# pierrepaleo/sift_pyocl

Measured on AMD Instinct MI355X. Metric: SiftPlan.keypoints throughput, 4096x4096 fp32 (Mpix/s; keypoints/s in keypoints_per_s), higher is better.
Workload: dtype f32

## Files before the change

sift_pyocl_amd/csrc/k_keypoint.hpp:

```cpp
#pragma once
#include <hip/hip_runtime.h>
#include <stdint.h>
#include "k_extrema.hpp"
#include "siftmath.hpp"

namespace siftk {

struct KpRecord { float x, y, scale, angle; uint8_t desc[128]; };
static_assert(sizeof(KpRecord) == 144, "record layout");

struct GradTaps { float xa, xb, ya, yb; bool bx, by; };

__device__ __forceinline__ GradTaps gradient_fetch(const float *__restrict__ I, int x, int y, int W, int H) {
    const size_t pos = (size_t)y * W + x;
    GradTaps t;
    t.bx = (x == 0) || (x == W - 1);
    t.by = (y == 0) || (y == H - 1);
    t.xa = I[x == W - 1 ? pos : pos + 1];
    t.xb = I[x == 0 ? pos : pos - 1];
    t.ya = I[y == 0 ? pos : pos - W];
    t.yb = I[y == H - 1 ? pos : pos + W];
    return t;
}

__device__ __forceinline__ void gradient_eval(const GradTaps &t, float &mag, float &ori) {
    float gx = t.xa - t.xb, gy = t.ya - t.yb;
    if (t.bx) gx = 2.0f * gx;
    if (t.by) gy = 2.0f * gy;
    mag = sqrtf(gx * gx + gy * gy);
    ori = siftmath::atan2f_(-gy, gx);
}

__device__ __forceinline__ void gradient_at(const float *__restrict__ I, int x, int y, int W, int H,
                                            float &mag, float &ori) {
    gradient_eval(gradient_fetch(I, x, y, W, H), mag, ori);
}

__device__ __forceinline__ int div_exact(int idx, int d, float inv, int &rem) {
    int q = (int)((float)idx * inv);
    rem = idx - q * d;
    if (rem < 0) { q--; rem += d; }
    else if (rem >= d) { q++; rem -= d; }
    return q;
}

#define SIFT_MAX_OCTAVES 24
#define SIFT_GROUPS 3
struct Counters {
    int n_rec;
    int tail_timeout;
    unsigned rec_word[SIFT_GROUPS];
    int g_kp[SIFT_GROUPS];
    int g_out[SIFT_GROUPS];
    int desc_next[SIFT_GROUPS];
    int n_cand[SIFT_MAX_OCTAVES + 1];
    int c_scale[SIFT_MAX_OCTAVES][3];
    int o_scale[SIFT_MAX_OCTAVES][3];
    uint32_t mm[2];
    int tail_ready[8];
};

struct OctaveTable {
    const float *base;
    long long off[SIFT_MAX_OCTAVES];
    int W[SIFT_MAX_OCTAVES], H[SIFT_MAX_OCTAVES];
    const float *gmap, *omap;
};
__device__ __forceinline__ size_t map_offset(const OctaveTable &tab, int oct, int scale) {
    return (size_t)(tab.off[oct] / 2) + (size_t)(scale - 1) * tab.W[oct] * tab.H[oct];
}

struct alignas(16) RecordSink {
    KpRecord *dev, *host;
    int dev_limit, host_limit;
};

__device__ __forceinline__ void descriptor_open(Counters *cnt, int group, int n, KpRecord *records, int rec_capacity, KpRecord *host_records,
                                                int host_capacity, RecordSink *S) {
    if (threadIdx.x == 0) {
        int base = 0;
        if (cnt) {
            if (blockIdx.x == 0) {
                base = atomicAdd(&cnt->n_rec, n);
                __hip_atomic_store(&cnt->rec_word[group], 0x80000000u | (unsigned)base, __ATOMIC_RELAXED, __HIP_MEMORY_SCOPE_AGENT);
            } else {
                unsigned w;
                while (!((w = __hip_atomic_load(&cnt->rec_word[group], __ATOMIC_RELAXED, __HIP_MEMORY_SCOPE_AGENT)) & 0x80000000u)) __builtin_amdgcn_s_sleep(16);
                base = (int)(w & 0x7fffffffu);
            }
        }
        S->dev = records + base; S->dev_limit = rec_capacity - base;
        S->host = host_records ? host_records + base : nullptr; S->host_limit = host_records ? host_capacity - base : 0;
    }
    __syncthreads();
}

__device__ __forceinline__ void store_record(const RecordSink *S, int i, const float4 kq, int b0, int b1, int lane, unsigned char *bytes) {
    bytes[lane] = (unsigned char)b0; bytes[lane + 64] = (unsigned char)b1;
    __builtin_amdgcn_wave_barrier();
    unsigned w = 0u;
    if (lane < 4) w = __float_as_uint(lane == 0 ? kq.x : (lane == 1 ? kq.y : (lane == 2 ? kq.z : kq.w)));
    else if (lane < 36) w = reinterpret_cast<const unsigned *>(bytes)[lane - 4];
    if (lane < 36) {
        const volatile RecordSink *v = S;
        if (i < v->dev_limit) reinterpret_cast<unsigned *>(v->dev + i)[lane] = w;
        if (i < v->host_limit) reinterpret_cast<unsigned *>(v->host + i)[lane] = w;
    }
    __builtin_amdgcn_wave_barrier();
}

__global__ void gather_records_kernel(const KpRecord *__restrict__ records, const int *__restrict__ idx, KpRecord *__restrict__ out, int n) {
    const long long total = (long long)n * 36;
    for (long long t = (long long)blockIdx.x * blockDim.x + threadIdx.x; t < total; t += (long long)gridDim.x * blockDim.x) {
        const int j = (int)(t / 36), w = (int)(t - (long long)j * 36);
        reinterpret_cast<unsigned *>(out + j)[w] = reinterpret_cast<const unsigned *>(records + idx[j])[w];
    }
}

#ifdef SIFT_PHASE_CLOCK
__device__ unsigned long long g_phase[32];
struct PhaseClock {
    unsigned long long t, t0;
    unsigned long long *acc;
    __device__ __forceinline__ void start(unsigned long long *lds16, int lane) {
        acc = lds16;
        if (lane < 16) lds16[lane] = 0ull;
        __builtin_amdgcn_wave_barrier();
        t0 = t = __builtin_amdgcn_s_memtime();
    }
    __device__ __forceinline__ void mark(int k, int lane) {
        const unsigned long long now = __builtin_amdgcn_s_memtime();
        if (lane == 0) (void)__hip_atomic_fetch_add(acc + k, now - t, __ATOMIC_RELAXED, __HIP_MEMORY_SCOPE_WORKGROUP);
        t = now;
    }
    __device__ __forceinline__ void count(int k, int lane) { if (lane == 0) (void)__hip_atomic_fetch_add(acc + k, 1ull, __ATOMIC_RELAXED, __HIP_MEMORY_SCOPE_WORKGROUP); }
    __device__ __forceinline__ void flush(int base, int lane) {
        const unsigned long long now = __builtin_amdgcn_s_memtime();
        if (lane == 0) acc[12] = now - t0;
        __builtin_amdgcn_wave_barrier();
        if (lane < 15) atomicAdd(&g_phase[base + lane], acc[lane]);
        if (lane == 15) atomicMax(&g_phase[base + 15], acc[12]);
    }
};
#define PH_MARK(k) ph.mark((k), lane)
#define PH_COUNT(k) ph.count((k), lane)
#define PH_WAIT_VM(n) asm volatile("s_waitcnt vmcnt(" #n ")" ::: "memory")
#else
#define PH_MARK(k)
#define PH_COUNT(k)
#define PH_WAIT_VM(n)
#endif

#define ABL(x) false

#define SIFT_ORI_OBUF 96
struct alignas(16) OriWaveLds {
    float pool[64 + 36 * 3 + 4];
    uint2 mask[36];
    unsigned mbase[36];
    float4 obuf[SIFT_ORI_OBUF];
    int oaux[SIFT_ORI_OBUF];
#ifdef SIFT_PHASE_CLOCK
    unsigned long long ph[16];
#endif
};

__device__ __forceinline__ int wave_prefix_incl(int x) {
    int t = x;
    t += __builtin_amdgcn_update_dpp(0, t, 0x111, 0xf, 0xf, false);
    t += __builtin_amdgcn_update_dpp(0, t, 0x112, 0xf, 0xf, false);
    t += __builtin_amdgcn_update_dpp(0, t, 0x114, 0xf, 0xf, false);
    t += __builtin_amdgcn_update_dpp(0, t, 0x118, 0xf, 0xf, false);
    t += __builtin_amdgcn_update_dpp(0, t, 0x142, 0xa, 0xf, false);
    t += __builtin_amdgcn_update_dpp(0, t, 0x143, 0xc, 0xf, false);
    return t;
}

template <bool MAPS>
__global__ __launch_bounds__(256) void orientation_kernel(OctaveTable tab, float ori_sigma,
                                                          const float4 *__restrict__ kp,
                                                          const int *__restrict__ kp_aux, Counters *cnt, int group,
                                                          int kp_capacity, float4 *__restrict__ okp,
                                                          int *__restrict__ oaux, int out_capacity, int team_below, int small_blocks) {
    __shared__ OriWaveLds lds_all[4];
    __shared__ double fold[36];
    __shared__ int s_hist[3 * SIFT_MAX_OCTAVES];
    const int lane = threadIdx.x & 63;
    OriWaveLds &L = lds_all[threadIdx.x >> 6];
    const int n = min(cnt->g_kp[group], kp_capacity);
    const int first = 0;
    const int count = n - first;
    const int nblocks = min((int)gridDim.x, count < 16384 ? small_blocks : (count < 65536 ? max(1024, small_blocks) : 4096));
    if ((int)blockIdx.x >= nblocks) return;
#ifdef SIFT_PHASE_CLOCK
    PhaseClock ph;
    ph.start(L.ph, lane);
#endif
    siftmath::load_atan_fold(fold);
    if (lane < 36) L.mask[lane] = make_uint2(0u, 0u);
    if (threadIdx.x < 3 * SIFT_MAX_OCTAVES) s_hist[threadIdx.x] = 0;
    __syncthreads();
    PH_MARK(0);
    const int wave = (blockIdx.x * blockDim.x + threadIdx.x) >> 6;
    const int nwaves = (nblocks * blockDim.x) >> 6;
    const float4 *pool4 = reinterpret_cast<const float4 *>(L.pool);
    __shared__ int s_pending[4], s_base;
    int pending = 0;
    auto store_pending = [&](int slot, int count) {
        __builtin_amdgcn_wave_barrier();
        for (int e = lane; e < count; e += 64)
            if (slot + e < out_capacity) { okp[slot + e] = L.obuf[e]; oaux[slot + e] = L.oaux[e]; }
        __builtin_amdgcn_wave_barrier();
    };
    auto flush_wave = [&]() {
        int slot = 0;
        if (lane == 0) slot = atomicAdd(&cnt->g_out[group], pending);
        store_pending(__shfl(slot, 0), pending);
        pending = 0;
    };
    const bool team = count < team_below;
    const int w4 = threadIdx.x >> 6;
    const int boff = team ? 64 * w4 : 0, bstep = team ? 256 : 64;
    for (int i = first + (team ? (int)blockIdx.x : wave); i < n; i += (team ? nblocks : nwaves)) {
        const float4 k = kp[i];
        const int aux = __builtin_amdgcn_readfirstlane(kp_aux[i]);
        const int scale = aux & 0xff, oct = aux >> 8;
        const int W = tab.W[oct], H = tab.H[oct], octsize = 1 << oct;
        if (!(k.y >= 0.0f)) continue;
        const float *I = tab.base + tab.off[oct] + (size_t)scale * W * H;
        const float *Gm = MAPS ? tab.gmap + map_offset(tab, oct, scale) : nullptr;
        const float *Om = MAPS ? tab.omap + map_offset(tab, oct, scale) : nullptr;
        auto taps_at = [&](int x, int y) {
            if (!MAPS) return gradient_fetch(I, x, y, W, H);
            GradTaps t = {};
            const size_t pos = (size_t)y * W + x;
            t.xa = Gm[pos]; t.xb = Om[pos];
            return t;
        };
        const int row = (int)((double)k.y + 0.5), col = (int)((double)k.z + 0.5);
        const float sigma = ori_sigma * k.w;
        const int radius = (int)((double)sigma * 3.0);
        const int rmin = max(0, row - radius), cmin = max(0, col - radius);
        const int rmax = min(row + radius, H - 2), cmax = min(col + radius, W - 2);
        const float lim = (float)(radius * radius) + 0.5f;
        const float two_s2 = 2.0f * sigma * sigma;
        const float r_two_s2 = 1.0f / two_s2;
        const bool fast_div = two_s2 >= 1e-3f && two_s2 <= 1e6f;
        const int wc = cmax - cmin + 1, hr = rmax - rmin + 1;
        const int total = (wc > 0 && hr > 0) ? wc * hr : 0;
        const float inv_wc = 1.0f / (float)max(wc, 1);
        float h = 0.0f;
        auto locate = [&](int base, int &r, int &c) {
            const int idx = base + lane;
            if (idx >= total) return false;
            int rem;
            const int q = div_exact(idx, wc, inv_wc, rem);
            r = rmin + q; c = cmin + rem;
            return true;
        };
        int nr = 0, nc = 0;
        bool nvalid = locate(boff, nr, nc);
        GradTaps ntaps = {};
        if (nvalid) ntaps = taps_at(nc, nr);
        PH_COUNT(13);
        PH_MARK(1);
        for (int base = 0; base < total; base += bstep) {
            bool valid = nvalid;
            const int r = nr, c = nc;
            const GradTaps taps = ntaps;
            nvalid = locate(base + bstep + boff, nr, nc);
            if (nvalid) ntaps = taps_at(nc, nr);
#ifdef SIFT_PHASE_CLOCK
            PH_COUNT(14);
            if (base + bstep + boff < total) PH_WAIT_VM(4); else PH_WAIT_VM(0);
            PH_MARK(2);
#endif
            int bin = 0;
            float val = 0.0f;
            if (valid) {
                float gx = taps.xa - taps.xb, gy = taps.ya - taps.yb;
                if (taps.bx) gx = 2.0f * gx;
                if (taps.by) gy = 2.0f * gy;
                const float gval = MAPS ? taps.xa : sqrtf(gx * gx + gy * gy);
                float dif = (float)r - k.y;
                float distsq = dif * dif;
                dif = (float)c - k.z;
                distsq = distsq + dif * dif;
                valid = (gval > 0.0f) && (distsq < lim);
                if (valid) {
                    const float earg = fast_div ? siftmath::div_by_reciprocal(-distsq, two_s2, r_two_s2) : -distsq / two_s2;
                    bool ok_a = true, ok_e;
                    float a = MAPS ? taps.xb : siftmath::atan2f_fast_try(-gy, gx, fold, ok_a);
                    float ew = siftmath::expf_fast_try(earg, ok_e);
                    if (!(ok_a && ok_e)) {
                        if (!MAPS && !ok_a) a = siftmath::atan2f_(-gy, gx);
                        if (!ok_e) ew = siftmath::expf_(earg);
                    }
                    bin = (int)siftmath::div_by_reciprocal(36.0f * (a + SM_PI_F + 0.001f), 2.0f * SM_PI_F, 1.0f / (2.0f * SM_PI_F));
                    valid = (bin >= 0) && (bin <= 36);
                    bin = min(max(bin, 0), 35);
                    val = ew * gval;
                }
                if (valid) atomicOr(reinterpret_cast<unsigned *>(L.mask) + 2 * bin + (lane >> 5), 1u << (lane & 31));
            }
            __builtin_amdgcn_wave_barrier();
            PH_MARK(3);
            const uint2 mine = (lane < 36) ? L.mask[lane] : make_uint2(0u, 0u);
            const int votes = __popc(mine.x) + __popc(mine.y);
            const int padded = (votes + 3) & ~3;
            const int seg = wave_prefix_incl(padded) - padded;
            if (lane < 36) L.mbase[lane] = (unsigned)seg;
            if (votes) reinterpret_cast<float4 *>(L.pool)[(seg + padded - 4) >> 2] = make_float4(0.f, 0.f, 0.f, 0.f);
            __builtin_amdgcn_wave_barrier();
            PH_MARK(4);
            {
                const uint2 mk = L.mask[bin];
                const unsigned mb = L.mbase[bin];
                const int pos = mb + __builtin_amdgcn_mbcnt_hi(mk.y, __builtin_amdgcn_mbcnt_lo(mk.x, 0u));
                if (valid) L.pool[pos] = val;
            }
            __builtin_amdgcn_wave_barrier();
            PH_MARK(5);
            if (!team) {
                for (int k0 = 0; k0 < padded; k0 += 4) {
                    const float4 v = pool4[(seg + k0) >> 2];
                    h = h + v.x; h = h + v.y; h = h + v.z; h = h + v.w;
                }
                if (votes) L.mask[lane] = make_uint2(0u, 0u);
                __builtin_amdgcn_wave_barrier();
                PH_MARK(6);
            } else {
                __syncthreads();
                if (w4 == 0 && lane < 36) {
#pragma unroll
                    for (int q = 0; q < 4; q++) {
                        const uint2 mq = lds_all[q].mask[lane];
                        const int vq = __popc(mq.x) + __popc(mq.y);
                        const int sq = (int)lds_all[q].mbase[lane];
                        const float4 *pq = reinterpret_cast<const float4 *>(lds_all[q].pool);
                        for (int k0 = 0; k0 < vq; k0 += 4) {
                            const float4 v = pq[(sq + k0) >> 2];
                            h = h + v.x; h = h + v.y; h = h + v.z; h = h + v.w;
                        }
                        if (vq) lds_all[q].mask[lane] = make_uint2(0u, 0u);
                    }
                }
                __syncthreads();
            }
        }
        if (team && w4 != 0) continue;
        const int lp = (lane == 0) ? 35 : lane - 1, ln = (lane >= 35) ? 0 : lane + 1;
        auto third = [&](float s) {
            return (__builtin_fabsf(s) >= 1e-25f && __builtin_fabsf(s) <= 1e30f) ? siftmath::div_by_reciprocal(s, 3.0f, 1.0f / 3.0f)
                                                                            : (float)((double)s / 3.0);
        };
#pragma unroll 1
        for (int pass = 0; pass < 6; pass++) {
            const float prev = __shfl(h, lp), nxt = __shfl(h, ln);
            float nh = third((prev + h) + nxt);
            const float nh0 = __shfl(nh, 0);
            if (lane == 35) nh = third((prev + h) + nh0);
            h = (lane < 36) ? nh : 0.0f;
        }
        float mx = (lane < 36) ? h : 0.0f;
#pragma unroll
        for (int off = 32; off > 0; off >>= 1) mx = fmaxf(mx, __shfl_xor(mx, off));
        const float maxval = fmaxf(mx, 0.0f);
        const uint64_t eq = __ballot(lane < 36 && h == maxval);
        const int argmax = (maxval > 0.0f && eq) ? (__ffsll((unsigned long long)eq) - 1) : 0;
        const float hp = __shfl(h, argmax == 0 ? 35 : argmax - 1);
        const float hn = __shfl(h, argmax == 35 ? 0 : argmax + 1);
        const float interp = 0.5f * (hp - hn) / (hp - 2.0f * maxval + hn);
        const float angle = 2.0f * SM_PI_F * ((float)argmax + 0.5f + interp) / 36.0f - SM_PI_F;
        const float hpp = __shfl(h, lp), hnn = __shfl(h, ln);
        bool extra = (lane < 36) && h > hpp && h > hnn && h >= 0.8f * maxval && lane != argmax;
        float a2 = 0.0f;
        if (extra) {
            const float it = 0.5f * (hpp - hnn) / (hpp - 2.0f * h + hnn);
            a2 = (float)((double)(2.0f * SM_PI_F * ((float)lane + 0.5f + it)) / 36.0 - (double)SM_PI_F);
            extra = (a2 >= -SM_PI_F) && (a2 <= SM_PI_F);
        }
        const uint64_t emask = __ballot(extra);
        const float ox = k.z * (float)octsize, oy = k.y * (float)octsize, os = k.w * (float)octsize;
        const float sum4 = ((ox + oy) + os) + angle;
        const int nmain = (sum4 == sum4) ? 1 : 0;
        const int nextra = __popcll((unsigned long long)emask);
        if (lane == 0) atomicAdd(&s_hist[3 * oct + min(max(scale - 1, 0), 2)], 1 + nextra);
        if (pending + nmain + nextra > SIFT_ORI_OBUF) flush_wave();
        if (lane == 0 && nmain) { L.obuf[pending] = make_float4(ox, oy, os, angle); L.oaux[pending] = aux; }
        if (extra) {
            const int at = pending + nmain + __popcll((unsigned long long)(emask & ((1ull << lane) - 1ull)));
            L.obuf[at] = make_float4(ox, oy, os, a2);
            L.oaux[at] = aux;
        }
        pending += nmain + nextra;
        PH_MARK(7);
    }
    if (lane == 0) s_pending[threadIdx.x >> 6] = pending;
    __syncthreads();
    if (threadIdx.x == 0) {
        const int tot = s_pending[0] + s_pending[1] + s_pending[2] + s_pending[3];
        s_base = tot ? atomicAdd(&cnt->g_out[group], tot) : 0;
    }
    __syncthreads();
    {
        const int w = threadIdx.x >> 6;
        int slot = s_base;
        for (int q = 0; q < w; q++) slot += s_pending[q];
        store_pending(slot, pending);
    }
    for (int t = threadIdx.x; t < 3 * SIFT_MAX_OCTAVES; t += blockDim.x)
        if (s_hist[t]) atomicAdd(&cnt->o_scale[0][0] + t, s_hist[t]);
#ifdef SIFT_PHASE_CLOCK
    PH_MARK(8);
    ph.flush(0, lane);
#endif
}


struct DescWaveLds {
    unsigned int mlo[128], mhi[128], mbase[128];
    float pool[8 * 64];
    int pool_cnt;
    int sij[128];
    float srx[128], scx[128];
    float V[128];
};

__global__ __launch_bounds__(256) __attribute__((amdgpu_waves_per_eu(4, 8))) void descriptor_stream_kernel(OctaveTable tab, const float4 *__restrict__ okp,
                                                         const int *__restrict__ oaux, Counters *cnt, int group,
                                                         int range_start, int range_end,
                                                         int out_capacity, KpRecord *__restrict__ records, int rec_capacity,
                                                         KpRecord *host_records, int host_capacity) {
    __shared__ DescWaveLds lds_all[4];
    __shared__ RecordSink sink;
    const int lane = threadIdx.x & 63, wave = threadIdx.x >> 6;
    DescWaveLds &L = lds_all[wave];
    int start = range_start, end = range_end;
    if (cnt) { start = 0; end = min(cnt->g_out[group], out_capacity); }
    descriptor_open(cnt, group, end, records, rec_capacity, host_records, host_capacity, &sink);
    L.mlo[lane] = 0u; L.mhi[lane] = 0u; L.mlo[lane + 64] = 0u; L.mhi[lane + 64] = 0u;
    if (lane == 0) L.pool_cnt = 0;
    const int gwave = blockIdx.x * 4 + wave, nwaves = gridDim.x * 4;
    const unsigned long long lt_mask = (1ull << lane) - 1ull;
    for (int i = start + gwave; i < end; i += nwaves) {
        const float4 kq = okp[i];
        const int aux = oaux[i];
        const int scale = aux & 0xff, oct = aux >> 8;
        const int W = tab.W[oct], H = tab.H[oct], octsize = 1 << oct;
        if (!(kq.y >= 0.0f)) {
            store_record(&sink, i, kq, 0, 0, lane, reinterpret_cast<unsigned char *>(L.V));
            continue;
        }
        const float *I = tab.base + tab.off[oct] + (size_t)scale * W * H;
        const float foct = (float)octsize;
        const float row = kq.y / foct, col = kq.x / foct, angle = kq.w;
        const int irow = (int)(row + 0.5f), icol = (int)(col + 0.5f);
        float sine, cosine;
        siftmath::sincosf_(angle, &sine, &cosine);
        const float spacing = kq.z / foct * 3.0f;
        const int iradius = (int)((1.414f * spacing * 2.5f) + 0.5f);
        const float drow = row - (float)irow, dcol = col - (float)icol;
        const int S = 2 * iradius + 1;
        const int total = S * S;
        const float inv_S = 1.0f / (float)S;
        float acc0 = 0.0f, acc1 = 0.0f;
        int list_n = 0, pos = 0;
        while (pos < total || list_n > 0) {
            while (list_n < 64 && pos < total) {
                const int idx = pos + lane;
                bool inside = false;
                float rx = 0.f, cx = 0.f;
                int ii = 0, jj = 0;
                if (idx < total) {
                    int rem;
                    const int q = div_exact(idx, S, inv_S, rem);
                    ii = q - iradius; jj = rem - iradius;
                    rx = ((cosine * (float)ii - sine * (float)jj) - drow) / spacing + 1.5f;
                    cx = ((sine * (float)ii + cosine * (float)jj) - dcol) / spacing + 1.5f;
                    const int yy = irow + ii, xx = icol + jj;
                    inside = rx > -1.0f && rx < 4.0f && cx > -1.0f && cx < 4.0f && yy >= 0 && yy < H && xx >= 0 && xx < W;
                }
                const unsigned long long bal = __ballot(inside);
                if (inside) {
                    const int at = list_n + __popcll(bal & lt_mask);
                    L.sij[at] = (ii + 32768) | ((jj + 32768) << 16);
                    L.srx[at] = rx;
                    L.scx[at] = cx;
                }
                list_n += __popcll(bal);
                pos += 64;
            }
            __builtin_amdgcn_wave_barrier();
            const int m = min(list_n, 64);
            int cbin[8];
            float cval[8];
#pragma unroll
            for (int n8 = 0; n8 < 8; n8++) { cbin[n8] = -1; cval[n8] = 0.0f; }
            if (lane < m && !ABL(3)) {
                const int pk = L.sij[lane];
                const int ii = (pk & 0xffff) - 32768, jj = ((pk >> 16) & 0xffff) - 32768;
                const float rx = L.srx[lane], cx = L.scx[lane];
                float g, o;
                if (ABL(2)) { g = I[(size_t)(irow + ii) * W + icol + jj]; o = g * 0.01f; }
                else gradient_at(I, icol + jj, irow + ii, W, H, g, o);
                const float er = rx - 1.5f, ec = cx - 1.5f;
                const float mag = g * (ABL(2) ? (er * ec) : siftmath::expf_(-0.125f * (er * er + ec * ec)));
                o = o - angle;
                while (o > 2.0f * SM_PI_F) o -= 2.0f * SM_PI_F;
                while (o < 0.0f) o += 2.0f * SM_PI_F;
                const float oval = 4.0f * o * SM_1_PI_F;
                const int ri = (int)((rx >= 0.0f) ? rx : rx - 1.0f);
                const int ci = (int)((cx >= 0.0f) ? cx : cx - 1.0f);
                const int oi = (int)((oval >= 0.0f) ? oval : oval - 1.0f);
                const float rf = rx - (float)ri, cf = cx - (float)ci, of = oval - (float)oi;
                const bool contributes = ri >= -1 && ri < 4 && oi >= 0 && oi <= 8 && rf >= 0.0f && rf <= 1.0f;
                if (contributes) {
                    const unsigned int bit = 1u << (lane & 31);
                    const int word = lane >> 5;
#pragma unroll
                    for (int a = 0; a < 2; a++) {
                        const int rb = ri + a;
                        const float rw = mag * (a == 0 ? 1.0f - rf : rf);
#pragma unroll
                        for (int bb = 0; bb < 2; bb++) {
                            const int cb = ci + bb;
                            const float cw = rw * (bb == 0 ? 1.0f - cf : cf);
                            const bool ok = rb >= 0 && rb < 4 && cb >= 0 && cb < 4;
#pragma unroll
                            for (int e = 0; e < 2; e++) {
                                int ob = oi + e;
                                const bool dup = (e == 1 && oi == 8);
                                if (ob >= 8) ob = 0;
                                const int n8 = a * 4 + bb * 2 + e;
                                if (ok && !dup) {
                                    cbin[n8] = (rb * 4 + cb) * 8 + ob;
                                    cval[n8] = cw * (e == 0 ? 1.0f - of : of);
                                    atomicOr((word ? L.mhi : L.mlo) + cbin[n8], bit);
                                }
                            }
                        }
                    }
                }
            }
            __builtin_amdgcn_wave_barrier();
            if (!(ABL(1) || ABL(3))) {
                const uint2 ia = make_uint2(L.mlo[lane], L.mhi[lane]), ib = make_uint2(L.mlo[lane + 64], L.mhi[lane + 64]);
                const int cnta = __popc(ia.x) + __popc(ia.y), cntb = __popc(ib.x) + __popc(ib.y);
                int base_a = 0;
                if (cnta + cntb) base_a = atomicAdd(&L.pool_cnt, cnta + cntb);
                const int base_b = base_a + cnta;
                if (cnta) L.mbase[lane] = (unsigned)base_a;
                if (cntb) L.mbase[lane + 64] = (unsigned)base_b;
                __builtin_amdgcn_wave_barrier();
                const unsigned lo_mask = (lane < 32) ? ((1u << lane) - 1u) : 0xffffffffu;
                const unsigned hi_mask = (lane < 32) ? 0u : ((1u << (lane - 32)) - 1u);
#pragma unroll
                for (int n8 = 0; n8 < 8; n8++)
                    if (cbin[n8] >= 0) {
                        const int b = cbin[n8];
                        L.pool[L.mbase[b] + __popc(L.mlo[b] & lo_mask) + __popc(L.mhi[b] & hi_mask)] = cval[n8];
                    }
                __builtin_amdgcn_wave_barrier();
                const int nmax = max(cnta, cntb);
                for (int r0 = 0; r0 < nmax; r0 += 4) {
                    float va[4], vb[4];
#pragma unroll
                    for (int u = 0; u < 4; u++) {
                        const float ra = L.pool[(base_a + r0 + u) & 511], rb_ = L.pool[(base_b + r0 + u) & 511];
                        va[u] = (r0 + u < cnta) ? ra : 0.0f;
                        vb[u] = (r0 + u < cntb) ? rb_ : 0.0f;
                    }
#pragma unroll
                    for (int u = 0; u < 4; u++) { acc0 = acc0 + va[u]; acc1 = acc1 + vb[u]; }
                }
                __builtin_amdgcn_wave_barrier();
                if (cnta) { L.mlo[lane] = 0u; L.mhi[lane] = 0u; }
                if (cntb) { L.mlo[lane + 64] = 0u; L.mhi[lane + 64] = 0u; }
                if (lane == 0) L.pool_cnt = 0;
            } else {
                L.mlo[lane] = 0u; L.mhi[lane] = 0u; L.mlo[lane + 64] = 0u; L.mhi[lane + 64] = 0u;
            }
            __builtin_amdgcn_wave_barrier();
            const int rest = list_n - m;
            int mij = 0; float mrx = 0.f, mcx = 0.f;
            if (lane < rest) { mij = L.sij[m + lane]; mrx = L.srx[m + lane]; mcx = L.scx[m + lane]; }
            __builtin_amdgcn_wave_barrier();
            if (lane < rest) { L.sij[lane] = mij; L.srx[lane] = mrx; L.scx[lane] = mcx; }
            list_n = rest;
            __builtin_amdgcn_wave_barrier();
        }
        L.V[lane] = acc0; L.V[lane + 64] = acc1;
        __builtin_amdgcn_wave_barrier();
        float norm = 0.0f;
#pragma unroll 8
        for (int k2 = 0; k2 < 128; k2++) { const float t = L.V[k2]; norm = norm + t * t; }
        norm = 1.0f / sqrtf(norm);
        acc0 = acc0 * norm; acc1 = acc1 * norm;
        const bool ch = (acc0 > 0.2f) || (acc1 > 0.2f);
        if (acc0 > 0.2f) acc0 = 0.2f;
        if (acc1 > 0.2f) acc1 = 0.2f;
        __builtin_amdgcn_wave_barrier();
        L.V[lane] = acc0; L.V[lane + 64] = acc1;
        __builtin_amdgcn_wave_barrier();
        if (__ballot(ch)) {
            float n2 = 0.0f;
#pragma unroll 8
            for (int k2 = 0; k2 < 128; k2++) { const float t = L.V[k2]; n2 = n2 + t * t; }
            n2 = 1.0f / sqrtf(n2);
            acc0 = acc0 * n2; acc1 = acc1 * n2;
        }
        __builtin_amdgcn_wave_barrier();
        const int i0 = (acc0 == acc0) ? (int)(512.0 * (double)acc0) : 0;
        const int i1 = (acc1 == acc1) ? (int)(512.0 * (double)acc1) : 0;
        store_record(&sink, i, kq, min(255, i0), min(255, i1), lane, reinterpret_cast<unsigned char *>(L.V));
    }
}

__global__ void gradient_kernel(const float *__restrict__ img, float *__restrict__ grad, float *__restrict__ ori, int W, int H) {
    const int x = blockIdx.x * blockDim.x + threadIdx.x, y = blockIdx.y;
    if (x >= W || y >= H) return;
    float g, o;
    gradient_at(img, x, y, W, H, g, o);
    grad[(size_t)y * W + x] = g;
    ori[(size_t)y * W + x] = o;
}

#define SIFT_MAP_ROWS 32
__host__ __device__ inline long long gradient_map_items_of(int W, int H) {
    return 3LL * ((H + SIFT_MAP_ROWS - 1) / SIFT_MAP_ROWS) * ((W + 255) / 256);
}
__global__ __launch_bounds__(256) void gradient_maps_kernel(OctaveTable tab, int oct_lo, int oct_hi, long long total,
                                                            float *__restrict__ gmap, float *__restrict__ omap) {
    __shared__ double fold[36];
    siftmath::load_atan_fold(fold);
    __syncthreads();
    for (long long item = blockIdx.x; item < total; item += gridDim.x) {
        long long rem = item;
        int oct = oct_lo;
        while (oct < oct_hi - 1 && rem >= gradient_map_items_of(tab.W[oct], tab.H[oct])) { rem -= gradient_map_items_of(tab.W[oct], tab.H[oct]); oct++; }
        const int W = tab.W[oct], H = tab.H[oct];
        const int nx = (W + 255) / 256, nyp = (H + SIFT_MAP_ROWS - 1) / SIFT_MAP_ROWS;
        const int plane = (int)(rem / ((long long)nyp * nx));
        const int r2 = (int)(rem - (long long)plane * nyp * nx);
        const int cy = r2 / nx, xb = r2 - cy * nx;
        if (plane > 2) continue;
        const int x = xb * 256 + (int)threadIdx.x;
        if (x >= W) continue;
        const float *I = tab.base + tab.off[oct] + (size_t)(plane + 1) * W * H;
        const size_t mo = map_offset(tab, oct, plane + 1);
        const int y1 = min((cy + 1) * SIFT_MAP_ROWS, H);
        for (int y = cy * SIFT_MAP_ROWS; y < y1; y++) {
            const GradTaps t = gradient_fetch(I, x, y, W, H);
            float gx = t.xa - t.xb, gy = t.ya - t.yb;
            if (t.bx) gx = 2.0f * gx;
            if (t.by) gy = 2.0f * gy;
            bool ok;
            float a = siftmath::atan2f_fast_try(-gy, gx, fold, ok);
            if (!ok) a = siftmath::atan2f_(-gy, gx);
            gmap[mo + (size_t)y * W + x] = sqrtf(gx * gx + gy * gy);
            omap[mo + (size_t)y * W + x] = a;
        }
    }
}

__global__ void math_kernel(int fn, const float *__restrict__ a, const float *__restrict__ bb, float *__restrict__ out, int64_t n) {
    __shared__ double fold[36];
    siftmath::load_atan_fold(fold);
    __syncthreads();
    const int64_t stride = (int64_t)gridDim.x * blockDim.x;
    for (int64_t i = (int64_t)blockIdx.x * blockDim.x + threadIdx.x; i < n; i += stride) {
        float s, c;
        switch (fn) {
            case 0: out[i] = siftmath::expf_(a[i]); break;
            case 1: out[i] = siftmath::exp2f_(a[i]); break;
            case 2: siftmath::sincosf_(a[i], &s, &c); out[i] = s; break;
            case 3: siftmath::sincosf_(a[i], &s, &c); out[i] = c; break;
            case 5: out[i] = siftmath::expf_fast(a[i]); break;
            case 6: out[i] = siftmath::atan2f_fast(a[i], bb[i], fold); break;
            case 7: out[i] = siftmath::div_by_reciprocal(a[i], bb[i], 1.0f / bb[i]); break;
            default: out[i] = siftmath::atan2f_(a[i], bb[i]); break;
        }
    }
}

}
```

Baseline: 21810.

## Restrict orientation sampling to circular row spans and add chunked dynamic keypoint scheduling

The orientation kernel now computes, for each row in the window, the column span that can fall inside the circular radius. It compacts these spans with a wave prefix sum and an LDS row table plus bitmask, so lanes only visit pixels near the circle rather than the full square. Non-team waves now fetch keypoints in chunks from a per-group atomic ticket counter instead of a static stride, to balance load. The cost is extra LDS, ballots, atomics and readlanes per keypoint. The new counter must start at zero for the scheduling to be correct.

```diff
diff --git a/sift_pyocl_amd/csrc/k_keypoint.hpp b/sift_pyocl_amd/csrc/k_keypoint.hpp
--- a/sift_pyocl_amd/csrc/k_keypoint.hpp
+++ b/sift_pyocl_amd/csrc/k_keypoint.hpp
@@ -53,6 +53,7 @@
     int g_kp[SIFT_GROUPS];
     int g_out[SIFT_GROUPS];
     int desc_next[SIFT_GROUPS];
+    int ori_next[SIFT_GROUPS];
     int n_cand[SIFT_MAX_OCTAVES + 1];
     int c_scale[SIFT_MAX_OCTAVES][3];
     int o_scale[SIFT_MAX_OCTAVES][3];
@@ -154,12 +155,18 @@
 #define ABL(x) false
 
 #define SIFT_ORI_OBUF 96
+#define SIFT_ORI_MAXRAD 31
+#ifndef SIFT_ORI_CHUNK
+#define SIFT_ORI_CHUNK 2
+#endif
 struct alignas(16) OriWaveLds {
     float pool[64 + 36 * 3 + 4];
     uint2 mask[36];
     unsigned mbase[36];
     float4 obuf[SIFT_ORI_OBUF];
     int oaux[SIFT_ORI_OBUF];
+    unsigned rowtab[64];
+    unsigned rowbits[128];
 #ifdef SIFT_PHASE_CLOCK
     unsigned long long ph[16];
 #endif
@@ -219,9 +226,23 @@
         pending = 0;
     };
     const bool team = count < team_below;
-    const int w4 = threadIdx.x >> 6;
+    const int w4 = __builtin_amdgcn_readfirstlane(threadIdx.x >> 6);
     const int boff = team ? 64 * w4 : 0, bstep = team ? 256 : 64;
-    for (int i = first + (team ? (int)blockIdx.x : wave); i < n; i += (team ? nblocks : nwaves)) {
+    const int chunk = count < 16384 ? SIFT_ORI_CHUNK : 2 * SIFT_ORI_CHUNK;
+    int chunk_left = 0;
+    int ticket = 0;
+    auto request = [&]() {
+        if (!team && chunk != 0 && chunk_left == 0 && lane == 0) ticket = atomicAdd(&cnt->ori_next[group], chunk);
+    };
+    auto advance = [&](int i) {
+        if (team) return i + nblocks;
+        if (chunk == 0) return i + nwaves;
+        if (chunk_left > 0) { chunk_left--; return i + 1; }
+        chunk_left = chunk - 1;
+        return first + nwaves + __builtin_amdgcn_readfirstlane(ticket);
+    };
+    for (int i = first + (team ? (int)blockIdx.x : wave); i < n; i = advance(i)) {
+        request();
         const float4 k = kp[i];
         const int aux = __builtin_amdgcn_readfirstlane(kp_aux[i]);
         const int scale = aux & 0xff, oct = aux >> 8;
@@ -247,12 +268,50 @@
         const float r_two_s2 = 1.0f / two_s2;
         const bool fast_div = two_s2 >= 1e-3f && two_s2 <= 1e6f;
         const int wc = cmax - cmin + 1, hr = rmax - rmin + 1;
-        const int total = (wc > 0 && hr > 0) ? wc * hr : 0;
         const float inv_wc = 1.0f / (float)max(wc, 1);
         float h = 0.0f;
+        const bool rows = radius <= SIFT_ORI_MAXRAD && W <= 65536;
+        int total = (wc > 0 && hr > 0) ? wc * hr : 0;
+        unsigned bits_lo = 0u, bits_hi = 0u;
+        int bits_before = 0;
+        if (rows) {
+            int len = 0, c0 = 0;
+            if (lane < hr && wc > 0) {
+                const float dr = (float)(rmin + lane) - k.y;
+                const float t = lim - dr * dr;
+                if (t > -1.0f) {
+                    const float w = sqrtf(fmaxf(t, 0.0f));
+                    const int lo = max((int)ceilf(k.z - w) - 1, cmin), hi = min((int)floorf(k.z + w) + 1, cmax);
+                    c0 = lo - cmin;
+                    len = max(hi - lo + 1, 0);
+                }
+            }
+            const int incl = wave_prefix_incl(len);
+            const int start = incl - len;
+            total = __builtin_amdgcn_readlane(incl, 63);
+            L.rowbits[lane] = 0u; L.rowbits[lane + 64] = 0u;
+            __builtin_amdgcn_wave_barrier();
+            const uint64_t filled = __ballot(len > 0);
+            if (len > 0) {
+                const int at = __builtin_amdgcn_mbcnt_hi((unsigned)(filled >> 32), __builtin_amdgcn_mbcnt_lo((unsigned)filled, 0u));
+                L.rowtab[at] = ((unsigned)start << 16) | ((unsigned)lane << 8) | (unsigned)c0;
+                if (start > 0) atomicOr(&L.rowbits[(start - 1) >> 5], 1u << ((start - 1) & 31));
+            }
+            __builtin_amdgcn_wave_barrier();
+            bits_lo = L.rowbits[2 * lane]; bits_hi = L.rowbits[2 * lane + 1];
+            const int nb = __popc(bits_lo) + __popc(bits_hi);
+            bits_before = wave_prefix_incl(nb) - nb;
+        }
         auto locate = [&](int base, int &r, int &c) {
             const int idx = base + lane;
             if (idx >= total) return false;
+            if (rows) {
+                const int b = base >> 6;
+                const unsigned lo = __builtin_amdgcn_readlane(bits_lo, b), hi = __builtin_amdgcn_readlane(bits_hi, b);
+                const unsigned word = L.rowtab[__builtin_amdgcn_mbcnt_hi(hi, __builtin_amdgcn_mbcnt_lo(lo, (unsigned)__builtin_amdgcn_readlane(bits_before, b)))];
+                r = rmin + (int)((word >> 8) & 0xffu); c = cmin + (int)(word & 0xffu) + (idx - (int)(word >> 16));
+                return true;
+            }
             int rem;
             const int q = div_exact(idx, wc, inv_wc, rem);
             r = rmin + q; c = cmin + rem;
```

Result: slower. 21070 (-3.4%).
